# hydradarpa/kalman-hydra

Hardware: AMD Instinct MI355X
Metric: frames/sec (Brox flow + EKF update) at 1024^2 (higher is better)
Workload: dtype f32 (flow, renders) / f64 (EKF sums and state)

## Files before the change

### include/hydra_mi.h

```cpp
#ifndef HYDRA_MI_H
#define HYDRA_MI_H

#include <stdint.h>

#ifdef __cplusplus
extern "C" {
#endif

#define HM_OK 0
#define HM_ERR_ARG (-1)
#define HM_ERR_HIP (-2)
#define HM_ERR_STATE (-3)
#define HM_ERR_NUMERIC (-4)

const char *hm_last_error(void);
const char *hm_version(void);
int hm_device_count(void);

int hm_dev_alloc(int device, uint64_t bytes, void **out);
int hm_dev_free(int device, void *ptr);
int hm_dev_upload(int device, void *dst, const void *src, uint64_t bytes);
int hm_dev_download(int device, void *dst, const void *src, uint64_t bytes);
int hm_copy_stream_create(int device, void **stream_out);
int hm_copy_stream_destroy(int device, void *stream);
// ... 80 lines not shown
                  double reltol, int info[4], double *errs, double *Hzc, double *gains, double *W_out);
int hm_cov_fetch(hm_ctx_t h, double *W_out);
int hm_ms_newton(int n_vertices, int n_bars, const int32_t *bars, const double *l0, double kappa, double M,
                 double dt, int maxiter, double tol, double *X, int *newton_iterations);
int hm_ms_worker_create(void **worker);
int hm_ms_worker_destroy(void *worker);
int hm_ms_newton_start(void *worker, int n_vertices, int n_bars, const int32_t *bars, const double *l0, double kappa,
                       double M, double dt, int maxiter, double tol, const double *X);
int hm_ms_newton_finish(void *worker, double *X, int *newton_iterations);
int hm_ms_worker_attach(void *worker, hm_ctx_t ctx);
int hm_newton_dev_start(hm_ctx_t h, int N, int n_bars, const int32_t *bars, const double *l0, double kappa, double M,
                        double dt, int maxiter, double tol, const double *X);
int hm_newton_dev_finish(hm_ctx_t h, double *X, int *newton_iterations);
int hm_update_arm_newton(hm_ctx_t h, void *worker, int n_bars, const int32_t *bars, const double *l0, double kappa,
                         double M, double dt, int maxiter, double tol);
int hm_update_arm_cov(hm_ctx_t h, double eps_F);
int hm_predict_take(hm_ctx_t h, const double *X, int n_bars, const int32_t *bars, const double *l0, double kappa,
                    double a, double s, double eps_F);
int hm_cov_predict(hm_ctx_t h, const double *W_in, int n_bars, const int32_t *bars, const double *blocks,
                   double a, double s, double eps_F, double *W_out);
int hm_ms_predict(hm_ctx_t h, int n_bars, const int32_t *bars, const double *l0, double kappa, double M, double dt,
                  int maxiter, double tol, double eps_F, double *X, int *newton_iterations, int prefactor);
int hm_update_last_error(hm_ctx_t h, const double *X, double err[4]);
int hm_chain_project(hm_ctx_t h);
int hm_prepare_mask(hm_ctx_t h, const uint8_t *d_y_m);
int hm_update_arm_mask(hm_ctx_t h, const uint8_t *d_y_m);
int hm_update_tail(hm_ctx_t h, double *Hzc, double *gains);
int hm_chain_states(hm_ctx_t h, double *predicted, double *projected, int *newton_iterations, int *moved);
int hm_ctx_tune(hm_ctx_t h, const char *key, int value);
int hm_ctx_tune64(hm_ctx_t h, const char *key, int64_t value);
int hm_ctx_sync(hm_ctx_t h);
void *hm_ctx_stream(hm_ctx_t h);

typedef struct hm_smooth *hm_smooth_t;
int hm_smooth_create(hm_ctx_t ctx, int capacity, int n_bars, const int32_t *bars, const double *l0, double kappa,
                     double a, double s, double eps_F, hm_smooth_t *out);
int hm_smooth_destroy(hm_smooth_t sm);
int hm_smooth_record(hm_smooth_t sm, const double *X);
int hm_smooth_run(hm_smooth_t sm, int want_cov, double *xs, double *var);
int hm_smooth_count(hm_smooth_t sm, int *frames, int *capacity);
int hm_smooth_fetch(hm_smooth_t sm, int k, double *P_out, double *x_out, double *m_out);
int hm_smooth_prior(hm_smooth_t sm, int k, double *Pp_out);
int hm_op_smooth_gemm(int device, int which, int n, const double *A, const double *B, const double *C, double *out);

int hm_view(hm_ctx_t h, const double *X, int which, const int32_t *palette, uint8_t *bgr);
int hm_view_dev(hm_ctx_t h, const double *X, int which, const int32_t *palette, void *d_bgr, void *stream);
// ... 118 lines not shown
```

### kalman-hydra_amd/_lib.py

```python
import ctypes
import os

import numpy as np

_HERE = os.path.dirname(os.path.abspath(__file__))
SO_PATH = os.environ.get("HYDRA_MI_SO") or os.path.join(_HERE, "libhydra_mi.so")

c_f32p = ctypes.POINTER(ctypes.c_float)
c_f64p = ctypes.POINTER(ctypes.c_double)
c_u8p = ctypes.POINTER(ctypes.c_uint8)
c_i32p = ctypes.POINTER(ctypes.c_int32)
c_vp = ctypes.c_void_p

SIGNATURES = {
    "hm_last_error": (ctypes.c_char_p, []),
    "hm_version": (ctypes.c_char_p, []),
    "hm_device_count": (ctypes.c_int, []),
    "hm_dev_alloc": (ctypes.c_int, [ctypes.c_int, ctypes.c_uint64, ctypes.POINTER(c_vp)]),
    "hm_dev_free": (ctypes.c_int, [ctypes.c_int, c_vp]),
    "hm_dev_upload": (ctypes.c_int, [ctypes.c_int, c_vp, c_vp, ctypes.c_uint64]),
    "hm_dev_download": (ctypes.c_int, [ctypes.c_int, c_vp, c_vp, ctypes.c_uint64]),
    "hm_copy_stream_create": (ctypes.c_int, [ctypes.c_int, ctypes.POINTER(c_vp)]),
    "hm_copy_stream_destroy": (ctypes.c_int, [ctypes.c_int, c_vp]),
    "hm_copy_stream_sync": (ctypes.c_int, [ctypes.c_int, c_vp]),
# ... 31 lines not shown
    "hm_op_sor": (ctypes.c_int, [c_vp, c_vp, ctypes.POINTER(c_vp), ctypes.c_int, ctypes.c_int, ctypes.c_int,
                                 ctypes.c_int, ctypes.c_float]),
    "hm_ctx_create": (ctypes.c_int, [ctypes.c_int, ctypes.c_int, ctypes.c_int, ctypes.c_int, ctypes.c_int, c_vp,
                                     c_vp, ctypes.c_double, ctypes.c_double, ctypes.c_double, ctypes.POINTER(c_vp)]),
    "hm_ctx_destroy": (ctypes.c_int, [c_vp]),
    "hm_set_texture": (ctypes.c_int, [c_vp, c_vp]),
    "hm_set_observation": (ctypes.c_int, [c_vp, c_vp, c_vp, c_vp, c_vp]),
    "hm_set_observation_dev": (ctypes.c_int, [c_vp, c_vp, c_vp, c_vp, c_vp]),
    "hm_render": (ctypes.c_int, [c_vp, c_vp, c_vp, c_vp, c_vp, c_vp]),
    "hm_initjacobian": (ctypes.c_int, [c_vp, c_vp, ctypes.c_int]),
    "hm_jz": (ctypes.c_int, [c_vp, c_vp, ctypes.c_int, c_f64p, c_f64p]),
    "hm_j": (ctypes.c_int, [c_vp, c_vp, ctypes.c_double, ctypes.c_int, ctypes.c_int, c_f64p]),
    "hm_jz_multi": (ctypes.c_int, [c_vp, c_vp, ctypes.c_int, c_vp, ctypes.c_int, c_vp, c_vp]),
    "hm_j_multi": (ctypes.c_int, [c_vp, c_vp, ctypes.c_double, ctypes.c_int, c_vp, c_vp, ctypes.c_int, c_vp, c_vp, c_vp]),
    "hm_error": (ctypes.c_int, [c_vp, c_vp, ctypes.c_int, c_f64p, c_vp, c_vp]),
    "hm_measure": (ctypes.c_int, [c_vp, c_vp, ctypes.c_double, ctypes.c_int, c_vp, c_vp, c_vp]),
    "hm_update_begin": (ctypes.c_int, [c_vp, c_vp, c_vp]),
    "hm_update_step": (ctypes.c_int, [c_vp, c_vp, ctypes.c_double, ctypes.c_int, c_vp, c_vp, c_f64p]),
    "hm_update_cov": (ctypes.c_int, [c_vp, ctypes.c_int, c_vp]),
    "hm_update_prefactor": (ctypes.c_int, [c_vp]),
    "hm_update_run": (ctypes.c_int, [c_vp, c_vp, c_vp, ctypes.c_double, ctypes.c_int, ctypes.c_int, ctypes.c_double,
                                     ctypes.POINTER(ctypes.c_int), c_vp, c_vp, c_vp, c_vp]),
    "hm_update_last_error": (ctypes.c_int, [c_vp, c_vp, c_f64p]),
    "hm_cov_fetch": (ctypes.c_int, [c_vp, c_vp]),
    "hm_project_mask": (ctypes.c_int, [c_vp, c_vp, c_vp, c_vp]),
    "hm_cov_predict": (ctypes.c_int, [c_vp, c_vp, ctypes.c_int, c_vp, c_vp, ctypes.c_double, ctypes.c_double,
                                      ctypes.c_double, c_vp]),
    "hm_ms_newton": (ctypes.c_int, [ctypes.c_int, ctypes.c_int, c_vp, c_vp, ctypes.c_double, ctypes.c_double,
                                    ctypes.c_double, ctypes.c_int, ctypes.c_double, c_vp, ctypes.POINTER(ctypes.c_int)]),
    "hm_ms_worker_create": (ctypes.c_int, [ctypes.POINTER(c_vp)]),
    "hm_ms_worker_destroy": (ctypes.c_int, [c_vp]),
    "hm_ms_newton_start": (ctypes.c_int, [c_vp, ctypes.c_int, ctypes.c_int, c_vp, c_vp, ctypes.c_double, ctypes.c_double,
                                          ctypes.c_double, ctypes.c_int, ctypes.c_double, c_vp]),
    "hm_ms_newton_finish": (ctypes.c_int, [c_vp, c_vp, ctypes.POINTER(ctypes.c_int)]),
    "hm_ms_worker_attach": (ctypes.c_int, [c_vp, c_vp]),
    "hm_newton_dev_start": (ctypes.c_int, [c_vp, ctypes.c_int, ctypes.c_int, c_vp, c_vp, ctypes.c_double, ctypes.c_double,
                                           ctypes.c_double, ctypes.c_int, ctypes.c_double, c_vp]),
    "hm_newton_dev_finish": (ctypes.c_int, [c_vp, c_vp, ctypes.POINTER(ctypes.c_int)]),
    "hm_prune_mask": (ctypes.c_int, [c_vp, c_vp, c_vp]),
    "hm_chain_project": (ctypes.c_int, [c_vp]),
    "hm_prepare_mask": (ctypes.c_int, [c_vp, c_vp]),
    "hm_update_arm_mask": (ctypes.c_int, [c_vp, c_vp]),
    "hm_update_tail": (ctypes.c_int, [c_vp, c_vp, c_vp]),
    "hm_chain_states": (ctypes.c_int, [c_vp, c_vp, c_vp, ctypes.POINTER(ctypes.c_int), ctypes.POINTER(ctypes.c_int)]),
    "hm_update_arm_newton": (ctypes.c_int, [c_vp, c_vp, ctypes.c_int, c_vp, c_vp, ctypes.c_double, ctypes.c_double,
                                            ctypes.c_double, ctypes.c_int, ctypes.c_double]),
# ... 203 lines not shown
```

### kalman-hydra_amd/csrc/ctx.h

```cpp
#pragma once
#include "hm_common.h"
#include "hm_types.h"
#include <chrono>
#include <cmath>
#include <condition_variable>
#include <functional>
#include <mutex>
#include <thread>
#include <vector>

struct Helper {
    std::thread th;
    std::mutex m;
    std::condition_variable cv;
    std::function<int()> job;
    bool posted = false, busy = false, quit = false;
    int rc = HM_OK;
    char err[512] = "";
    void run()
    {
        std::unique_lock<std::mutex> lk(m);
        for (;;) {
            cv.wait(lk, [&] { return quit || posted; });
            if (quit) return;
// ... 24 lines not shown
        rc = HM_OK;
        return r;
    }
    void stop()
    {
        {
            std::unique_lock<std::mutex> lk(m);
            cv.wait(lk, [&] { return !busy; });
            quit = true;
            cv.notify_all();
        }
        if (th.joinable()) th.join();
    }
};

struct Armed {
    bool newton = false;
    void *worker = nullptr;
    bool cov = false;
    const uint8_t *mask = nullptr;
};

struct ViewState {
    Targets targets = {nullptr, nullptr, nullptr, nullptr};
    TriSetup *setup = nullptr;
    int *ids = nullptr, *lab = nullptr;
    unsigned *wire = nullptr, *mm = nullptr;
    double *X = nullptr, *force = nullptr;
    uint8_t *out = nullptr;
    hipEvent_t ev = nullptr;
    int c_layers = 0, c_L = 0;
    bool c_weighted = false;
    int *c_lab = nullptr;
    uint16_t *c_w = nullptr;
    uint8_t *c_col = nullptr;
    uint8_t *c_outline = nullptr;
    uint8_t *c_frame = nullptr;
    uint8_t *c_in = nullptr;
    uint8_t *c_slot[4] = {nullptr, nullptr, nullptr, nullptr};
    hipEvent_t c_slot_ev[4] = {nullptr, nullptr, nullptr, nullptr};
    bool c_slot_used[4] = {false, false, false, false};
    int c_next = 0;
};
#define VIEW_CELL_SLOTS 4

struct BodyState {
    bool ready = false;
// ... 92 lines not shown
    std::vector<double> resv, tailv;
    int result_delay = 0;
    bool tail_pending = false;
    bool tail_valid = false;
    long long tail_ticket = 0;
    hipStream_t tail_stream = nullptr;
    Armed armed;
    std::vector<int> sp_h_off, sp_h_bar, sp_h_other;
    std::vector<double> sp_h_blk;
    std::vector<int32_t> sp_bars_cached;
    std::vector<int> tri;
    DPool pool;
    int *d_area;
    int *d_sp_off, *d_sp_bar, *d_sp_other;
    double *d_sp_blk;
    bool upd_open;
    bool prefactored;
    std::vector<double> h_partial;
    int red_blocks = 512;
    double *d_tpart = nullptr;
    std::vector<double> h_tpart;
    int ntiles = 0;
    int render_rows = RI_H;
    bool last_err_valid = false;
    double last_err[4] = {0, 0, 0, 0};
    std::vector<double> last_err_X;
    long long run_ticket;
    int vsplit = 5, esplit;
    std::vector<int32_t> pn_bars;
    std::vector<double> pn_l0;
    double pn_par[4] = {0, 0, 0, 0};
    int pn_maxiter = 0;
    double pq_eps_F = 0.0;
    bool pq_valid = false;
    std::vector<double> pq_X, pq_l0;
    std::vector<int32_t> pq_bars;
    double pq_par[4] = {0, 0, 0, 0};
    hipStream_t stream3 = nullptr;
    int *d_n4nbr = nullptr, *d_n4nbb = nullptr, *d_n4bars = nullptr;
    double *d_n4l0 = nullptr;
    int n4deg = 0;
    std::vector<int32_t> n4_bars;
    std::vector<double> n4_l0;
    double *pin_n4 = nullptr;
    double *d_n4X = nullptr;
    std::vector<double> n4v;
// ... 30 lines not shown
    std::vector<double> h_lout;
    int2 *d_outline;
    int *d_outline_cnt;
    uint8_t *d_pm_mask;
    uint8_t *d_pm_flag = nullptr;
    uint8_t *d_pm_pruned = nullptr;
    Ccl ccl = {nullptr, nullptr, nullptr, nullptr, nullptr, 0, 0};
    double *d_pm_X = nullptr;
    double *pin_pm = nullptr;
    std::vector<double> pmv;
    int *d_pm_done = nullptr;
    long long pm_ticket = 0;
    bool pm_ready = false;
    bool outline_ready = false;
    const uint8_t *prepared_mask = nullptr;
    hipEvent_t ev_outline = nullptr;
    hipEvent_t ev_m0 = nullptr;
    ViewState view;
    BodyState body;
    StrainState strain;
    RecState rec;
};

static inline hipError_t alloc_targets(HmOwner &own, Targets &t, size_t n)
{
    hipError_t e = own.alloc(&t.acc, n * sizeof(int));
    if (e == hipSuccess) e = own.alloc(&t.fx, n * sizeof(float));
    if (e == hipSuccess) e = own.alloc(&t.fy, n * sizeof(float));
    if (e == hipSuccess) e = own.alloc(&t.cnt, n * sizeof(int));
    return e;
}

static int helper_join(hm_ctx *h)
{
    if (h->helper_used) {
        const int rc = h->helper.wait();
        if (rc != HM_OK) { hm_set_error("%s", h->helper.err); return rc; }
    }
    return HM_OK;
}
static int ctx_join(hm_ctx *h, bool lazy = false)
{
    if (!h) return HM_OK;
    if (const int rc = helper_join(h)) return rc;
    if (!lazy && h->tail_on_stream4) {
        h->tail_on_stream4 = false;
        if (hipSetDevice(h->device) != hipSuccess || hipStreamWaitEvent(h->stream, h->ev_tail, 0) != hipSuccess) {
            hm_set_error("the handle's stream cannot wait for the tail of the last update");
            return HM_ERR_HIP;
        }
    }
    if (h->worker_active) {
// ... 94 lines not shown
```

### kalman-hydra_amd/csrc/ekf.hip

```cpp
#include "ctx.h"
#include "ekf_kernels.h"
#include "dense_kernels.h"
#include "chol_flow_kernels.h"
#include "project_kernels.h"
#include "predict_kernels.h"
#include <algorithm>
#include <atomic>
#include <chrono>
#include <cmath>
#include <cstring>
#include <set>
#include <thread>
#include <utility>
#include <vector>


static int hb_wait(hipStream_t st, const double *blk, size_t first, size_t n, unsigned long long stamp, double *out, const char *who)
{
    const volatile unsigned long long *canary = (const volatile unsigned long long *)blk + 2 * (first + n - 1);
    const auto t_start = std::chrono::steady_clock::now();
    const auto t_yield = t_start + std::chrono::microseconds(700), t_give_up = t_start + std::chrono::milliseconds(20);
    bool polite = false;
    for (int spin = 0;; spin++) {
        if ((canary[0] ^ canary[1]) == stamp && hb_take(blk, first, n, stamp, out)) return HM_OK;
// ... 129 lines not shown
    hipError_t e = hipSuccess;
    auto dev = [&](auto **p, size_t bytes) { if (e == hipSuccess) e = h->own.alloc(p, bytes); };
    if (rc == HM_OK) {
        const char *pe = getenv("HYDRA_MI_EKF_PRIORITY");
        e = h->own.stream(&h->stream, !(pe && atoi(pe) == 0));
        dev(&h->d_tex, n);
        dev(&h->d_yim, n);
        dev(&h->d_ym, n);
        dev(&h->d_yfx, n * sizeof(float));
        dev(&h->d_yfy, n * sizeof(float));
        dev(&h->d_yfxm, n * sizeof(float));
        dev(&h->d_yfym, n * sizeof(float));
        dev(&h->d_setup, (size_t)T * sizeof(TriSetup));
        dev(&h->d_cfgs, (size_t)N * MEAS_NCFG * (EKF_MAX_STAR + 1) * sizeof(TriSetup));
        dev(&h->d_ubox, (size_t)N * UBOX_STRIDE * sizeof(int4));
        dev(&h->d_tmask, (size_t)N * TMASK_STRIDE * sizeof(unsigned));
        dev(&h->d_tlist, (size_t)N * TMASK_STRIDE * sizeof(int));
        dev(&h->d_tcount, (size_t)N * sizeof(int));
        dev(&h->d_X, (size_t)4 * N * sizeof(double));
        dev(&h->d_out, (size_t)h->njobs * MEAS_VSPLIT_MAX * MEAS_OUT * sizeof(double));
        dev(&h->d_partial, (size_t)h->red_blocks * 4 * sizeof(double));
        h->ntiles = hm_cdiv(W, RI_W) * hm_cdiv(H, 8);
        dev(&h->d_tpart, (size_t)h->ntiles * RI_NV * sizeof(double));
        dev(&h->d_im8, n);
        dev(&h->d_m8, n);
        const size_t n4 = (size_t)4 * N, nn = n4 * n4 * sizeof(double);
        dev(&h->d_H, nn);
        dev(&h->d_HTH, nn);
        if (e == hipSuccess) e = hipMemsetAsync(h->d_HTH, 0, nn, h->stream);
        dev(&h->d_invW0, nn);
        const size_t nn_aug = (size_t)(hm_cdiv((int)n4, DNB) * DNB + DNB) * n4 * sizeof(double);
        dev(&h->d_Af[0], nn_aug);
        dev(&h->d_Af[1], nn_aug);
        dev(&h->d_Awork, nn_aug);
        const size_t ld_bytes = (size_t)hm_cdiv((int)n4, DNB) * DNB * DNB * sizeof(double);
        dev(&h->d_T[0], nn);
        dev(&h->d_T[1], nn);
        dev(&h->d_step, n4 * sizeof(double));
        dev(&h->d_Lt[0], ld_bytes);
        dev(&h->d_Lt[1], ld_bytes);
        dev(&h->d_Wtmp, nn);
        dev(&h->d_flowP, 3 * ld_bytes);
        dev(&h->d_flowctl, 4 * sizeof(unsigned));
        if (e == hipSuccess) e = hipMemsetAsync(h->d_flowctl, 0, 4 * sizeof(unsigned), h->stream);
        dev(&h->d_Hz, n4 * sizeof(double));
        dev(&h->d_Hzc, n4 * 4 * sizeof(double));
        dev(&h->d_Wprior, nn);
        dev(&h->d_gain, n4 * 3 * sizeof(double));
        h->pin_n = 2 * (n4 + RES_HEAD + n4 * 4 + n4 * 3) + 2;
        if (e == hipSuccess) e = h->own.host_alloc(&h->pin, h->pin_n * sizeof(double), hipHostMallocCoherent);
        if (e == hipSuccess) memset(h->pin, 0, h->pin_n * sizeof(double));
        h->pin_scratch = (int *)(h->pin + h->pin_n - 2);
        h->resv.assign(n4 + RES_HEAD, 0.0);
        h->tailv.assign(n4 * 7, 0.0);
        dev(&h->d_X0, n4 * sizeof(double));
        dev(&h->pool.hdr, (size_t)4 * N * sizeof(int));
        dev(&h->pool.overflow, sizeof(int));
        dev(&h->d_area, (size_t)N * sizeof(int));
        h->pool.area = h->d_area;
        if (e == hipSuccess) e = pool_alloc(h, (long long)8 * W * H);
        dev(&h->d_Xn, n4 * sizeof(double));
        for (Targets *t : {&h->ref, &h->P, &h->Q})
            if (e == hipSuccess) e = alloc_targets(h->own, *t, n);
    }
    if (e != hipSuccess) {
        hm_set_error("hm_ctx_create: device allocation failed: %s", hipGetErrorString(e));
        step(HM_ERR_HIP);
    }
    if (rc != HM_OK) {
        ctx_free(h);
        return rc;
    }
    h->h_partial.resize((size_t)h->red_blocks * 4);
    h->h_tpart.resize((size_t)h->ntiles * RI_NV);
    *out = h;
    return HM_OK;
}

extern "C" int hm_ctx_destroy(hm_ctx_t h) { return ctx_free(h); }

void ekf_queue_setup_all(hipStream_t st, const Mesh &m, const double *d_X, TriSetup *d_setup)
{
    hipLaunchKernelGGL(k_setup_all, dim3(hm_cdiv(m.T, 64)), dim3(64), 0, st, m, d_X, d_setup);
}
void ekf_queue_render(hipStream_t st, const Mesh &m, const double *d_X, const TriSetup *d_setup, const Targets &out,
                      const int *d_labels, int *d_ids)
// ... 11 lines not shown
    return HM_OK;
}
#endif

#define TUNE_SET(field) [](hm_ctx *h, long long v) { h->field = (decltype(h->field))v; }
static const struct TuneKey {
    const char *key;
    long long lo, hi;
    int step;
    void (*set)(hm_ctx *, long long);
    const char *must;
} tune_keys[] = {
    {"measure_split", 1, MEAS_VSPLIT_MAX, 1, TUNE_SET(vsplit), nullptr},
    {"edge_split", 1, MEAS_VSPLIT_MAX, 1, TUNE_SET(esplit), nullptr},
    {"chol_flow", 0, 1, 1, TUNE_SET(chol_flow), "must be 0 (one launch per block step) or 1 (one persistent launch)"},
    {"chol_flow_wgs", 2, 2048, 1, TUNE_SET(flow_wgs), "must be in 2..2048 (the chain workgroup and at least one task workgroup)"},
    {"render_rows", 8, 16, 8, TUNE_SET(render_rows), "must be 8 or 16"},
    {"chol_flow_stall", 0, 100000, 1, TUNE_SET(flow_stall), nullptr},
    {"result_delay", 0, 5000, 1, TUNE_SET(result_delay), "must be in 0..5000 (microseconds)"},
    {"tail_async", 0, 1, 1, TUNE_SET(tail_async), "must be 0 or 1"},
    {"tail_split", 0, 1, 1, TUNE_SET(tail_split), "must be 0 or 1"},
    {"newton_fail", 0, 1, 1, TUNE_SET(newton_fail), "must be 0 or 1"},
    {"speculate", 0, 1, 1, TUNE_SET(speculate), "must be 0 or 1"},
    {"body_stats_cap", 1, BODY_STATS_CAP, 1, TUNE_SET(body.stats_cap), nullptr},
    {"body_rec_chunk", 0, INT32_MAX, 1, TUNE_SET(rec.chunk), "must be >= 0 (0: the default size)"},
    {"rec_tp_frames", 1, REC_TP_MAX, 1, TUNE_SET(rec.tp_frames), nullptr},
    {"rec_bl_frames", 1, REC_BL_MAX, 1, TUNE_SET(rec.bl_frames), nullptr},
    {"rec_res_frames", 1, REC_RES_MAX, 1, TUNE_SET(rec.res_frames), nullptr},
    {"rec_map_frames", 1, REC_MAP_MAX, 1, TUNE_SET(rec.map_frames), nullptr},
    {"rec_null_frames", 1, REC_NULL_MAX, 1, TUNE_SET(rec.null_frames), nullptr},
    {"rec_tm_frames", 1, REC_TM_MAX, 1, TUNE_SET(rec.tm_frames), nullptr},
    {"rec_gram_bytes", 64, REC_GRAM_BYTES_MAX, 64, TUNE_SET(rec.gram_bytes), "must be a multiple of 64 in 64..131008"},
    {"rec_scratch_bytes", 1, 1 << 30, 1, TUNE_SET(rec.scr_bytes), nullptr},
    {"rec_ev_bytes", 1, 1ll << 34, 1, TUNE_SET(rec.ev_bytes), nullptr},
};
#undef TUNE_SET
static const TuneKey *tune_find(const char *key)
{
    for (const TuneKey &k : tune_keys)
        if (!strcmp(key, k.key)) return &k;
    return nullptr;
}
static int tune_set(hm_ctx *h, const char *key, long long value)
{
    const TuneKey *k = tune_find(key);
    HM_ARG(k != nullptr, "hm_ctx_tune: unknown key '%s'", key);
// ... 78 lines not shown
    h->pm_ready = true;
    return HM_OK;
}
static int queue_outline(hm_ctx *h, const uint8_t *mask)
{
    HM_HIP(hipMemsetAsync(h->d_outline_cnt, 0, 4 * sizeof(int), h->stream2));
    const dim3 cg(hm_cdiv(h->W, 64), hm_cdiv(h->H, CCL_NT / 64)), cb(CCL_NT);
    hipLaunchKernelGGL(k_ccl_local, dim3(hm_cdiv(h->W, CCL_TW), hm_cdiv(h->H, CCL_TH)), cb, 0, h->stream2, mask, h->ccl);
    hipLaunchKernelGGL(k_ccl_border, cg, cb, 0, h->stream2, mask, h->ccl);
    hipLaunchKernelGGL(k_ccl_roots, cg, cb, 0, h->stream2, h->ccl);
    hipLaunchKernelGGL(k_ccl_flatten, cg, cb, 0, h->stream2, mask, h->ccl);
    hipLaunchKernelGGL(k_ccl_stats, cg, cb, 0, h->stream2, mask, h->ccl);
    hipLaunchKernelGGL(k_ccl_select, cg, cb, 0, h->stream2, mask, h->ccl);
    hipLaunchKernelGGL(k_ccl_write, cg, cb, 0, h->stream2, mask, h->ccl, h->d_pm_pruned);
    Outline o = {h->d_outline, h->d_outline_cnt, h->W * h->H, h->d_pm_flag};
    hipLaunchKernelGGL(k_outline, dim3(hm_cdiv(h->W, 64), hm_cdiv(h->H, OUTLINE_NT / 64)), dim3(OUTLINE_NT), 0, h->stream2,
                       (const uint8_t *)h->d_pm_pruned, h->W, h->H, o);
    HM_HIP(hipGetLastError());
    HM_HIP(hipEventRecord(h->ev_outline, h->stream2));
    h->prepared_mask = nullptr;
    return HM_OK;
}

static int finish_observation(hm_ctx *h)
{
    h->last_err_valid = false;
    const int n = h->W * h->H;
    hipLaunchKernelGGL(k_mask_flow, dim3(hm_cdiv(n, 256)), dim3(256), 0, h->stream, h->o_ym, h->o_yfx, h->o_yfy,
                       h->d_yfxm, h->d_yfym, n);
    HM_HIP(hipGetLastError());
    h->have_obs = true;
    return HM_OK;
}

extern "C" int hm_set_observation(hm_ctx_t h, const uint8_t *y_im, const float *y_fx, const float *y_fy,
                                  const uint8_t *y_m)
{
    HM_ARG(h && y_im && y_fx && y_fy && y_m, "hm_set_observation: NULL argument");
    HM_JOIN(h);
    HM_HIP(hipSetDevice(h->device));
    const size_t n = (size_t)h->W * h->H;
    HM_HIP(hipMemcpyAsync(h->d_yim, y_im, n, hipMemcpyHostToDevice, h->stream));
    HM_HIP(hipMemcpyAsync(h->d_ym, y_m, n, hipMemcpyHostToDevice, h->stream));
    HM_HIP(hipMemcpyAsync(h->d_yfx, y_fx, n * sizeof(float), hipMemcpyHostToDevice, h->stream));
    HM_HIP(hipMemcpyAsync(h->d_yfy, y_fy, n * sizeof(float), hipMemcpyHostToDevice, h->stream));
    h->o_yim = h->d_yim; h->o_ym = h->d_ym; h->o_yfx = h->d_yfx; h->o_yfy = h->d_yfy;
    HM_TRY(finish_observation(h));
    HM_HIP(hipStreamSynchronize(h->stream));
    h->outline_ready = false;
// ... 6 lines not shown

extern "C" int hm_set_observation_dev(hm_ctx_t h, const uint8_t *d_y_im, const float *d_y_fx, const float *d_y_fy,
                                      const uint8_t *d_y_m)
{
    HM_ARG(h && d_y_im && d_y_fx && d_y_fy && d_y_m, "hm_set_observation_dev: NULL argument");
    HM_JOIN_LAZY(h);
    HM_HIP(hipSetDevice(h->device));
    h->o_yim = d_y_im; h->o_ym = d_y_m; h->o_yfx = d_y_fx; h->o_yfy = d_y_fy;
    HM_TRY(finish_observation(h));
    h->outline_ready = false;
    if (h->d_outline && h->prepared_mask == d_y_m) {
        h->outline_ready = true;
    } else if (h->d_outline) {
        HM_TRY(queue_outline(h, h->o_ym));
        h->outline_ready = true;
    }
    h->prepared_mask = nullptr;
    return HM_OK;
}

static int render_dev(hm_ctx *h, const double *dX, Targets t)
{
    Mesh m = {h->W, h->H, h->N, h->T, h->d_tri, h->d_uv, h->d_tex};
    hipLaunchKernelGGL(k_setup_all, dim3(hm_cdiv(h->T, 64)), dim3(64), 0, h->stream, m, dX, h->d_setup);
    hipLaunchKernelGGL((k_render<0>), dim3(hm_cdiv(h->W, EKF_TILE), hm_cdiv(h->H, EKF_TILE)), dim3(EKF_TILE, EKF_TILE), 0,
                       h->stream, m, dX, h->d_setup, t, (const int *)nullptr, (int *)nullptr);
    HM_HIP(hipGetLastError());
    return HM_OK;
}

static int render_into(hm_ctx *h, const double *X, Targets t)
{
    HM_HIP(hipMemcpyAsync(h->d_X, X, (size_t)4 * h->N * sizeof(double), hipMemcpyHostToDevice, h->stream));
    return render_dev(h, h->d_X, t);
}

static void measure_args(hm_ctx *h, const double *dX, double deltaX, int masked, MeasureArgs &a);
static int render_strips(const hm_ctx *h) { return hm_cdiv(h->W, RI_W) * hm_cdiv(h->H, h->render_rows); }

static int render_iter(hm_ctx *h, const double *dX, Targets t, bool with_err, int masked, bool regions, double deltaX)
{
    IterRenderArgs r;
    r.m = Mesh{h->W, h->H, h->N, h->T, h->d_tri, h->d_uv, h->d_tex};
    r.X = dX;
    r.out = t;
    r.o = Obs{h->o_yim, masked ? h->d_yfxm : h->o_yfx, masked ? h->d_yfym : h->o_yfy, h->o_ym};
    r.raw_fx = h->o_yfx; r.raw_fy = h->o_yfy;
    r.partial = h->d_tpart;
    r.tiles_x = hm_cdiv(h->W, RI_W); r.tiles_y = hm_cdiv(h->H, h->render_rows);
    const int nstrips = r.tiles_x * r.tiles_y;
    r.with_err = with_err ? 1 : 0;
    r.n_regions = regions ? h->N : 0;
    MeasureArgs a;
    measure_args(h, dX, deltaX, masked, a);
    if (h->render_rows == 8) hipLaunchKernelGGL((k_render_iter<8>), dim3(r.n_regions + nstrips), dim3(256), 0, h->stream, r, a, h->d_area);
    else hipLaunchKernelGGL((k_render_iter<16>), dim3(r.n_regions + nstrips), dim3(256), 0, h->stream, r, a, h->d_area);
    HM_HIP(hipGetLastError());
    return HM_OK;
}

static void hm_tile_partial_sums(const double *p, int ntiles, double s[RI_NV])
{
    static thread_local double g[RI_GROUPS][RI_NV];
    for (int t = 0; t < RI_GROUPS; t++) {
        double a[RI_NV];
        for (int k = 0; k < RI_NV; k++) a[k] = 0.0;
        for (int i = t; i < ntiles; i += RI_GROUPS)
            for (int k = 0; k < RI_NV; k++) a[k] += p[RI_NV * (size_t)i + k];
        for (int k = 0; k < RI_NV; k++) g[t][k] = a[k];
    }
    for (int k = 0; k < RI_NV; k++) {
        double v = 0.0;
        for (int t = 0; t < RI_GROUPS; t++) v += g[t][k];
        s[k] = v;
    }
// ... 111 lines not shown
                const int v = h->tri[3 * t + k];
                const double x = states[sidx][2 * v], y = states[sidx][2 * v + 1];
                x0 = std::min(x0, x); x1 = std::max(x1, x); y0 = std::min(y0, y); y1 = std::max(y1, y);
            }
        if (!(x0 <= x1 && y0 <= y1)) continue;
        const int c0 = (int)std::max(0.0, std::floor(std::min(x0, (double)h->W)) - 1.0);
        const int c1 = (int)std::min((double)h->W - 1.0, std::ceil(std::max(x1, -1.0)) + 1.0);
        const int r0 = (int)std::max(0.0, std::floor(std::min(y0, (double)h->H)) - 1.0);
        const int r1 = (int)std::min((double)h->H - 1.0, std::ceil(std::max(y1, -1.0)) + 1.0);
        int4 &b = box[lab];
        if (b.x > b.y) b = make_int4(c0, c1, r0, r1);
        else b = make_int4(std::min(b.x, c0), std::max(b.y, c1), std::min(b.z, r0), std::max(b.w, r1));
    }
    HM_HIP(hipMemcpyAsync(h->d_labels, labels, (size_t)h->T * sizeof(int), hipMemcpyHostToDevice, h->stream));
    HM_HIP(hipMemcpyAsync(h->d_lbox, box.data(), (size_t)n_labels * sizeof(int4), hipMemcpyHostToDevice, h->stream));
    HM_HIP(hipStreamSynchronize(h->stream));
    return HM_OK;
}

static int render_ids(hm_ctx *h, const double *X, Targets t, int *ids, bool ids_only)
{
    HM_HIP(hipMemcpyAsync(h->d_X, X, (size_t)4 * h->N * sizeof(double), hipMemcpyHostToDevice, h->stream));
    Mesh m = {h->W, h->H, h->N, h->T, h->d_tri, h->d_uv, h->d_tex};
    hipLaunchKernelGGL(k_setup_all, dim3(hm_cdiv(h->T, 64)), dim3(64), 0, h->stream, m, h->d_X, h->d_setup);
    const dim3 grid(hm_cdiv(h->W, EKF_TILE), hm_cdiv(h->H, EKF_TILE)), block(EKF_TILE, EKF_TILE);
    if (ids_only) hipLaunchKernelGGL((k_render<2>), grid, block, 0, h->stream, m, h->d_X, h->d_setup, t, (const int *)h->d_labels, ids);
    else hipLaunchKernelGGL((k_render<1>), grid, block, 0, h->stream, m, h->d_X, h->d_setup, t, (const int *)h->d_labels, ids);
    HM_HIP(hipGetLastError());
    HM_HIP(hipStreamSynchronize(h->stream));
    return HM_OK;
}

extern "C" int hm_jz_multi(hm_ctx_t h, const double *Xp, int masked, const int32_t *labels, int n_labels, double *hz,
                           double *hzc)
{
    HM_ARG(h && Xp && labels && hz && n_labels >= 1, "hm_jz_multi: bad argument");
    HM_JOIN(h);
    NEED_REF(h, "hm_jz_multi");
    HM_HIP(hipSetDevice(h->device));
    const double *states[2] = {h->X0.data(), Xp};
    HM_TRY(multi_setup(h, labels, n_labels, states, 2));
    int rc = render_ids(h, h->X0.data(), h->ref, h->d_ids[0], true);
    if (rc == HM_OK) rc = render_ids(h, Xp, h->P, h->d_ids[1], false);
    if (rc) return rc;
    MultiArgs a = {h->ref, h->P, h->P, h->d_ids[0], h->d_ids[1], h->d_ids[1], obs_of(h, masked), h->W, h->d_lbox, h->d_lout};
    hipLaunchKernelGGL(k_jz_multi, dim3(n_labels), dim3(RED_NT), 0, h->stream, a);
// ... 837 lines not shown
        HM_TRY(update_queue_iteration(u, it, swap));
        HM_TRY(update_meanwhile(u, it));
        Taken taken = Taken::go_on;
        HM_TRY(update_take_result(u, it, swap, &taken));
        if (taken == Taken::retry) continue;
        Verdict verdict = Verdict::go_on;
        HM_TRY(update_judge(u, it, &verdict));
        if (verdict != Verdict::go_on) break;
        swap.keep();
        it++;
    }
    HM_TRY(update_state_final(u));
    HM_TRY(update_tail(u));
    update_finish(u, info);
    return HM_OK;
}

extern "C" int hm_update_last_error(hm_ctx_t h, const double *X, double err[4])
{
    HM_ARG(h && X && err, "hm_update_last_error: NULL argument");
    if (!h->last_err_valid || h->last_err_X.size() != (size_t)4 * h->N) return 1;
    if (memcmp(X, h->last_err_X.data(), (size_t)4 * h->N * sizeof(double)) != 0) return 1;
    for (int k = 0; k < 4; k++) err[k] = h->last_err[k];
    return HM_OK;
}

void ekf_queue_fpft(hipStream_t st, const double *src, double *FP, double *dst, int N, const SpringTopo &tp, double a, double s,
                    double eps_F)
{
    const dim3 grid(hm_cdiv(4 * N, 256), N);
    hipLaunchKernelGGL(k_fw_rows, grid, dim3(256), 0, st, src, FP, N, tp, a, s);
    hipLaunchKernelGGL(k_pft_cols, grid, dim3(256), 0, st, (const double *)FP, dst, N, tp, a, s, eps_F);
}
void ekf_queue_chol_flow(hipStream_t st, const FlowArgs &a, int wgs, bool fill)
{
    if (fill) hipLaunchKernelGGL(k_flow_fill, dim3(a.nrows + FLOW_FILL_WGS), dim3(256), 0, st, a);
    hipLaunchKernelGGL(k_chol_flow, dim3(wgs), dim3(FLOW_NT), 0, st, a);
}

static int cov_predict_core(hm_ctx *h, const double *W_in, int n_bars, const int32_t *bars, const double *blocks,
                            double a, double s, double eps_F, double *W_out, bool ahead, hipStream_t st = nullptr)
{
    if (!st) st = h->stream;
    const int N = h->N, n4 = 4 * N;
    const size_t nn = (size_t)n4 * n4 * sizeof(double);
    std::vector<int> &off = h->sp_h_off, &bar = h->sp_h_bar, &other = h->sp_h_other;
// ... 320 lines not shown
```

### kalman-hydra_amd/csrc/ekf_kernels.h

```cpp
#pragma once
#include <hip/hip_runtime.h>
#include <stdint.h>
#include "hm_types.h"

__global__ void k_setup_all(Mesh m, const double *__restrict__ X, TriSetup *__restrict__ out)
{
    int t = blockIdx.x * blockDim.x + threadIdx.x;
    if (t >= m.T) return;
    int v0 = m.tri[3 * t], v1 = m.tri[3 * t + 1], v2 = m.tri[3 * t + 2];
    TriSetup s;
    d_tri_setup(s, v0, v1, v2, d_snap(X[2 * v0]), d_snap(X[2 * v0 + 1]), d_snap(X[2 * v1]), d_snap(X[2 * v1 + 1]),
                d_snap(X[2 * v2]), d_snap(X[2 * v2 + 1]), m.W, m.H);
    d_tri_attr(s, m.uv, X, m.N);
    out[t] = s;
}

template <int MODE>
__global__ __launch_bounds__(EKF_TILE *EKF_TILE) void k_render(Mesh m, const double *__restrict__ X,
                                                                const TriSetup *__restrict__ setup, Targets out,
                                                                const int *__restrict__ labels, int *__restrict__ ids)
{
    __shared__ unsigned s_mask[EKF_MAX_TRI / 32];
    const int tid = threadIdx.y * EKF_TILE + threadIdx.x;
    const int words = (m.T + 31) / 32;
// ... 702 lines not shown
                acc[B_VXX] = fma(avx, bxfx, acc[B_VXX]); acc[B_VXY] = fma(avx, byfx, acc[B_VXY]);
                acc[B_VXVX] = fma(avx, bvx, acc[B_VXVX]);
                acc[B_XVY] = fma(axfy, bvy, acc[B_XVY]); acc[B_YVY] = fma(ayfy, bvy, acc[B_YVY]);
                acc[B_VYX] = fma(avy, bxfy, acc[B_VYX]); acc[B_VYY] = fma(avy, byfy, acc[B_VYY]);
                acc[B_VYVY] = fma(avy, bvy, acc[B_VYVY]);
            }
            if (!more) break;
        }
    }
    d_block_reduce<B_NV, MEAS_NT>(acc, s_red, a.out + ((size_t)(N + e) * MEAS_VSPLIT_MAX + blockIdx.y) * MEAS_OUT);
}

#define RI_CHUNK 32
#define RI_GROUPS 256
#define RI_W 64
struct IterRenderArgs {
    Mesh m;
    const double *X;
    Targets out;
    Obs o;
    const float *raw_fx, *raw_fy;
    double *partial;
    int tiles_x, tiles_y, with_err, n_regions;
};
#define RI_NV 6
struct RenderShared {
    unsigned mask[EKF_MAX_TRI / 32];
    TriSetup cand[RI_CHUNK];
    double red[(256 / 64) * RI_NV];
    unsigned band[RI_W / 8];
};

#ifdef HM_STAMP
__device__ long long *g_stamp;
#define HM_STAMP_AT(k) do { if (g_stamp && threadIdx.x == 0) g_stamp[(size_t)blockIdx.x * 8 + (k)] = wall_clock64(); } while (0)
#else
#define HM_STAMP_AT(k) do { } while (0)
#endif
template <int RIH>
__global__ __launch_bounds__(256, 4) void k_render_iter(IterRenderArgs r, MeasureArgs a, int *__restrict__ area)
{
    HM_STAMP_AT(0);
    constexpr int RI_PX = RI_W * RIH / 256;
    __shared__ union {
        RegionShared reg;
        RenderShared t;
// ... 16 lines not shown
        const bool has2 = tc < m.T;
        const int a0 = m.tri[3 * ta], a1 = m.tri[3 * ta + 1], a2 = m.tri[3 * ta + 2];
        const int b0 = has2 ? m.tri[3 * tc] : a0, b1 = has2 ? m.tri[3 * tc + 1] : a1, b2 = has2 ? m.tri[3 * tc + 2] : a2;
        const double ax0 = X[2 * a0], ay0 = X[2 * a0 + 1], ax1 = X[2 * a1], ay1 = X[2 * a1 + 1], ax2 = X[2 * a2], ay2 = X[2 * a2 + 1];
        const double bx0 = X[2 * b0], by0 = X[2 * b0 + 1], bx1 = X[2 * b1], by1 = X[2 * b1 + 1], bx2 = X[2 * b2], by2 = X[2 * b2 + 1];
#pragma unroll
        for (int k = 0; k < 2; k++) {
            if (k == 1 && !has2) break;
            const int t = k ? tc : ta;
            const double x0 = k ? bx0 : ax0, y0 = k ? by0 : ay0, x1 = k ? bx1 : ax1, y1 = k ? by1 : ay1, x2 = k ? bx2 : ax2, y2 = k ? by2 : ay2;
            const double lo_x = fmin(x0, fmin(x1, x2)) - 2.0, hi_x = fmax(x0, fmax(x1, x2)) + 2.0;
            const double lo_y = fmin(y0, fmin(y1, y2)) - 2.0, hi_y = fmax(y0, fmax(y1, y2)) + 2.0;
            if (hi_x < (double)c0 || lo_x > (double)(c0 + RI_W) || hi_y < (double)r0 || lo_y > (double)(r0 + RIH)) continue;
            int cmin, cmax, rmin, rmax;
            d_tri_bbox(d_snap(x0), d_snap(y0), d_snap(x1), d_snap(y1), d_snap(x2), d_snap(y2), m.W, m.H, cmin, cmax, rmin, rmax);
            if (cmin <= cmax && cmax >= c0 && cmin < c0 + RI_W && rmax >= r0 && rmin < r0 + RIH)
                atomicOr(&sh.t.mask[t >> 5], 1u << (t & 31));
        }
    }
    __syncthreads();
    HM_STAMP_AT(1);
    int total = 0;
    for (int w = 0; w < words; w++) total += __popc(sh.t.mask[w]);
    const int c = c0 + (tid & 63), rb = r0 + (tid >> 6);
    int acc[RI_PX], cnt[RI_PX], tadr[RI_PX];
    float fx[RI_PX], fy[RI_PX];
#pragma unroll
    for (int q = 0; q < RI_PX; q++) { acc[q] = 0; cnt[q] = 0; fx[q] = 0.0f; fy[q] = 0.0f; tadr[q] = -1; }
    for (int base = 0; base < total; base += RI_CHUNK) {
        const int nch = min(RI_CHUNK, total - base);
        for (int tb = tid; tb < m.T; tb += 256) {
            const unsigned word = sh.t.mask[tb >> 5], bit = 1u << (tb & 31);
            if (!(word & bit)) continue;
            int rank = __popc(word & (bit - 1u));
            for (int w = 0; w < (tb >> 5); w++) rank += __popc(sh.t.mask[w]);
            if (rank < base || rank >= base + nch) continue;
            const int v0 = m.tri[3 * tb], v1 = m.tri[3 * tb + 1], v2 = m.tri[3 * tb + 2];
            TriSetup su;
            d_tri_setup(su, v0, v1, v2, d_snap(X[2 * v0]), d_snap(X[2 * v0 + 1]), d_snap(X[2 * v1]), d_snap(X[2 * v1 + 1]),
                        d_snap(X[2 * v2]), d_snap(X[2 * v2 + 1]), m.W, m.H);
            d_tri_attr(su, m.uv, X, m.N);
            {
                const double xa = (double)c0, xb = (double)min(c0 + RI_W - 1, m.W - 1);
                const double ya = (double)r0, yb = (double)min(r0 + RIH - 1, m.H - 1);
                bool out = false;
#pragma unroll
// ... 39 lines not shown
                    if (tadr[j] < 0) tadr[j] = at;
                    else acc[j] += m.tex[at];
                    fx[j] = fx[j] + d_lerp(su.ax[0], su.ax[1], su.ax[2], l1, l2);
                    fy[j] = fy[j] + d_lerp(su.ay[0], su.ay[1], su.ay[2], l1, l2);
                    cnt[j]++;
                }
            }
        __syncthreads();
    }
    HM_STAMP_AT(2);
    {
        int tx[RI_PX];
#pragma unroll
        for (int j = 0; j < RI_PX; j++) tx[j] = m.tex[tadr[j] < 0 ? 0 : tadr[j]];
#pragma unroll
        for (int j = 0; j < RI_PX; j++) acc[j] += tadr[j] < 0 ? 0 : tx[j];
    }
    double e[RI_NV] = {0.0, 0.0, 0.0, 0.0, 0.0, 0.0};
#pragma unroll
    for (int j = 0; j < RI_PX; j++) {
        const int rr = rb + 4 * j;
        if (c >= m.W || rr >= m.H) continue;
        const int p = rr * m.W + c;
        r.out.acc[p] = acc[j]; r.out.fx[p] = fx[j]; r.out.fy[p] = fy[j]; r.out.cnt[p] = cnt[j];
        if (r.with_err) {
            const unsigned rim = acc[j] > 255 ? 255 : acc[j];
            const unsigned rm = cnt[j] > 0 ? 255 : 0;
            const unsigned d = ((unsigned)r.o.yim[p] - rim) & 255u;
            const unsigned dm = ((255u * (unsigned)r.o.ym[p]) - rm) & 255u;
            const float dfx = r.o.yfx[p] - fx[j];
            const float dfy = r.o.yfy[p] + fy[j];
            e[0] += (double)((d * d) & 255u);
            e[1] += (double)dfx * (double)dfx;
            e[2] += (double)dfy * (double)dfy;
            e[3] += (double)((dm * dm) & 255u);
            const float gfx = r.raw_fx[p] - fx[j];
            const float gfy = r.raw_fy[p] + fy[j];
            e[4] += (double)gfx * (double)gfx;
            e[5] += (double)gfy * (double)gfy;
        }
    }
    HM_STAMP_AT(3);
    if (!r.with_err) return;
    d_block_reduce<RI_NV, 256>(e, sh.t.red, r.partial + RI_NV * (size_t)tile);
    HM_STAMP_AT(4);
}

__device__ __forceinline__ void d_tile_partial_sums(const double *__restrict__ partial, int ntiles, double *sp, double *out)
{
    const int t = threadIdx.x;
    if (t < RI_GROUPS) {
        double s[RI_NV];
#pragma unroll
        for (int k = 0; k < RI_NV; k++) s[k] = 0.0;
#pragma unroll 4
        for (int i = t; i < ntiles; i += RI_GROUPS) {
            const double2 *q = (const double2 *)(partial + RI_NV * (size_t)i);
#pragma unroll
            for (int k = 0; k < RI_NV / 2; k++) { const double2 v = q[k]; s[2 * k] += v.x; s[2 * k + 1] += v.y; }
        }
#pragma unroll
        for (int k = 0; k < RI_NV; k++) sp[RI_NV * t + k] = s[k];
    }
    __syncthreads();
    if (t < RI_NV) {
        double s = 0.0;
// ... 92 lines not shown
```

### kalman-hydra_amd/csrc/hm_types.h

```cpp
#pragma once
#include <hip/hip_runtime.h>
#include <stdint.h>
#include <stddef.h>


#define EKF_SUB 256
#define EKF_MAX_STAR 24
#define EKF_TILE 16
#define EKF_MAX_TRI 4096

struct TriSetup {
    double ea[3], eb[3], ec[3];
    double ecb[3];
    int cmin, cmax, rmin, rmax;
    int tl[3];
    float inv;
    int i0, i1, i2;
    float ux[3], uy[3], ax[3], ay[3];
};

__device__ __forceinline__ void d_tri_attr(TriSetup &s, const float *__restrict__ uv, const double *__restrict__ X, int N)
{
    const int id[3] = {s.i0, s.i1, s.i2};
    for (int k = 0; k < 3; k++) {
// ... 114 lines not shown
    float ty = d_lerp(s.uy[0], s.uy[1], s.uy[2], l1, l2);
    int cx = (int)floorf(tx), cy = (int)floorf(ty);
    cx = cx < 0 ? 0 : (cx > W - 1 ? W - 1 : cx);
    cy = cy < 0 ? 0 : (cy > H - 1 ? H - 1 : cy);
    return cy * W + cx;
}
__device__ __forceinline__ int d_texel(const uint8_t *__restrict__ tex, const TriSetup &s, float l1, float l2, int W,
                                       int H)
{
    return tex[d_texel_at(s, l1, l2, W, H)];
}

struct Mesh {
    int W, H, N, T;
    const int *tri;
    const float *uv;
    const uint8_t *tex;
};

struct Targets {
    int *acc;
    float *fx, *fy;
    int *cnt;
};

struct DPool {
    int *hdr;
    int *live;
    const int *area;
    short2 *xi, *yi;
    float *xfx, *xfy, *yfx, *yfy, *vxfx, *vyfy;
    long long cap;
    int *overflow;
};

#define RI_H 16

#define DNB 32

typedef double d4_t __attribute__((ext_vector_type(4)));

__device__ __forceinline__ d4_t d_mfma_nn(double (*X)[DNB + 1], double (*Y)[DNB + 1], int wv, int lane, d4_t c)
{
    const int i = 16 * (wv >> 1) + (lane & 15), j = 16 * (wv & 1) + (lane & 15), kq = lane >> 4;
#pragma unroll
    for (int kk = 0; kk < DNB / 4; kk++)
// ... 83 lines not shown
```

### kalman-hydra_amd/renderer.py

```python
import ctypes
import os

import numpy as np

from . import _lib
from . import matio


class ChainedPredictionFailed(RuntimeError):
    """hm_update_run, chained to a state prediction on the device (hm_chain_project), found that the prediction's inner
    solve had given up: nothing was updated; predict on the host and update again."""


class Renderer:
    def __init__(self, distmesh, vel, flow, nx, im1, cuda, eps_Z, eps_J, eps_M, labels=None, labels_hess=None,
                 Q=None, showtracking=False, force=None, multi=True, device=0):
        if not cuda:
            raise NotImplementedError(
                "cuda=False: this build has no CPU measurement path (the reference's NumPy twin, "
                "cuda.py:929-1010, is restated under oracle/ as test infrastructure only)")
        self._h = None
        self.Q = Q
        self.cuda = cuda
        self.force = force
# ... 50 lines not shown
        self.velocities = np.asarray(velocities, np.float64).reshape(-1, 2)
        table = self.labels_hess if hess else self.labels
        if multi_idx is None or multi_idx < 0 or table is None:
            self._palette = None
        else:
            self._palette = np.ascontiguousarray(np.asarray(table)[:, multi_idx], np.int32)

    def _X(self, state=None):
        if state is not None:
            return np.ascontiguousarray(np.asarray(state.X, np.float64).reshape(-1))
        return np.ascontiguousarray(np.concatenate((self.vertices.reshape(-1), self.velocities.reshape(-1))))

    def render(self):
        n = self.nx * self.ny
        im = np.empty((self.ny, self.nx), np.uint8)
        m = np.empty_like(im)
        fx = np.empty((self.ny, self.nx), np.float32)
        fy = np.empty_like(fx)
        _lib.check(_lib.lib().hm_render(self._h, _lib.ptr(self._X()), _lib.ptr(im), _lib.ptr(fx), _lib.ptr(fy),
                                        _lib.ptr(m)), "hm_render")
        self.last_render = (im, fx, fy, m)
        return self.last_render

    def get_flow(self):
        _, fx, fy, _ = self.render()
        return fx, fy

    def _view_palette(self):
        lh = self.labels_hess
        if lh is None or np.ndim(lh) != 2 or np.shape(lh)[1] < 2:
            return None
        return np.ascontiguousarray(np.asarray(lh)[:, 1], np.int32)

    def view(self, X=None, which="overlay"):
        from .videoio import VIEWS
        x = self._X() if X is None else np.ascontiguousarray(np.asarray(X, np.float64).reshape(-1))
        if x.shape[0] != 4 * self.n:
            raise ValueError("state of %d entries for a mesh of %d vertices" % (x.shape[0], self.n))
        out = np.empty((self.ny, self.nx, 3), np.uint8)
        pal = self._view_palette() if which == "mask" else None
        _lib.check(_lib.lib().hm_view(self._h, _lib.ptr(x), VIEWS[which], _lib.ptr(pal), _lib.ptr(out)), "hm_view")
        return out

    def view_dev(self, X, which, d_out, stream=None):
        from .videoio import VIEWS
        x = np.ascontiguousarray(np.asarray(X, np.float64).reshape(-1))
# ... 863 lines not shown
```

Before: 335.8.

## Skip rewriting empty render tiles and reuse per-tile error partials across iterations

```diff
diff --git a/include/hydra_mi.h b/include/hydra_mi.h
--- a/include/hydra_mi.h
+++ b/include/hydra_mi.h
@@ -126,6 +126,7 @@
 int hm_ms_predict(hm_ctx_t h, int n_bars, const int32_t *bars, const double *l0, double kappa, double M, double dt,
                   int maxiter, double tol, double eps_F, double *X, int *newton_iterations, int prefactor);
 int hm_update_last_error(hm_ctx_t h, const double *X, double err[4]);
+int hm_targets_fetch(hm_ctx_t h, int which, int32_t *acc, float *fx, float *fy, int32_t *cnt);
 int hm_chain_project(hm_ctx_t h);
 int hm_prepare_mask(hm_ctx_t h, const uint8_t *d_y_m);
 int hm_update_arm_mask(hm_ctx_t h, const uint8_t *d_y_m);
diff --git a/kalman-hydra_amd/_lib.py b/kalman-hydra_amd/_lib.py
--- a/kalman-hydra_amd/_lib.py
+++ b/kalman-hydra_amd/_lib.py
@@ -77,6 +77,7 @@
     "hm_update_run": (ctypes.c_int, [c_vp, c_vp, c_vp, ctypes.c_double, ctypes.c_int, ctypes.c_int, ctypes.c_double,
                                      ctypes.POINTER(ctypes.c_int), c_vp, c_vp, c_vp, c_vp]),
     "hm_update_last_error": (ctypes.c_int, [c_vp, c_vp, c_f64p]),
+    "hm_targets_fetch": (ctypes.c_int, [c_vp, ctypes.c_int, c_vp, c_vp, c_vp, c_vp]),
     "hm_cov_fetch": (ctypes.c_int, [c_vp, c_vp]),
     "hm_project_mask": (ctypes.c_int, [c_vp, c_vp, c_vp, c_vp]),
     "hm_cov_predict": (ctypes.c_int, [c_vp, c_vp, ctypes.c_int, c_vp, c_vp, ctypes.c_double, ctypes.c_double,
diff --git a/kalman-hydra_amd/csrc/ctx.h b/kalman-hydra_amd/csrc/ctx.h
--- a/kalman-hydra_amd/csrc/ctx.h
+++ b/kalman-hydra_amd/csrc/ctx.h
@@ -70,7 +70,7 @@
 };
 
 struct ViewState {
-    Targets targets = {nullptr, nullptr, nullptr, nullptr};
+    Targets targets = {nullptr, nullptr, nullptr, nullptr, nullptr};
     TriSetup *setup = nullptr;
     int *ids = nullptr, *lab = nullptr;
     unsigned *wire = nullptr, *mm = nullptr;
@@ -209,6 +209,11 @@
     std::vector<double> h_tpart;
     int ntiles = 0;
     int render_rows = RI_H;
+    int render_skip = 1;
+    int *d_tstamp = nullptr;
+    int obs_epoch = 1;
+    bool skip_live = false;
+    int skip_rows = 0, skip_masked = -1;
     bool last_err_valid = false;
     double last_err[4] = {0, 0, 0, 0};
     std::vector<double> last_err_X;
@@ -285,12 +290,13 @@
     RecState rec;
 };
 
-static inline hipError_t alloc_targets(HmOwner &own, Targets &t, size_t n)
+static inline hipError_t alloc_targets(HmOwner &own, Targets &t, size_t n, size_t strips = 0)
 {
     hipError_t e = own.alloc(&t.acc, n * sizeof(int));
     if (e == hipSuccess) e = own.alloc(&t.fx, n * sizeof(float));
     if (e == hipSuccess) e = own.alloc(&t.fy, n * sizeof(float));
     if (e == hipSuccess) e = own.alloc(&t.cnt, n * sizeof(int));
+    if (e == hipSuccess && strips) e = own.alloc(&t.dirty, strips);
     return e;
 }
 
diff --git a/kalman-hydra_amd/csrc/ekf.hip b/kalman-hydra_amd/csrc/ekf.hip
--- a/kalman-hydra_amd/csrc/ekf.hip
+++ b/kalman-hydra_amd/csrc/ekf.hip
@@ -175,6 +175,7 @@
         dev(&h->d_partial, (size_t)h->red_blocks * 4 * sizeof(double));
         h->ntiles = hm_cdiv(W, RI_W) * hm_cdiv(H, 8);
         dev(&h->d_tpart, (size_t)h->ntiles * RI_NV * sizeof(double));
+        dev(&h->d_tstamp, (size_t)h->ntiles * sizeof(int));
         dev(&h->d_im8, n);
         dev(&h->d_m8, n);
         const size_t n4 = (size_t)4 * N, nn = n4 * n4 * sizeof(double);
@@ -214,7 +215,7 @@
         if (e == hipSuccess) e = pool_alloc(h, (long long)8 * W * H);
         dev(&h->d_Xn, n4 * sizeof(double));
         for (Targets *t : {&h->ref, &h->P, &h->Q})
-            if (e == hipSuccess) e = alloc_targets(h->own, *t, n);
+            if (e == hipSuccess) e = alloc_targets(h->own, *t, n, (size_t)h->ntiles);
     }
     if (e != hipSuccess) {
         hm_set_error("hm_ctx_create: device allocation failed: %s", hipGetErrorString(e));
@@ -272,6 +273,7 @@
     {"tail_split", 0, 1, 1, TUNE_SET(tail_split), "must be 0 or 1"},
     {"newton_fail", 0, 1, 1, TUNE_SET(newton_fail), "must be 0 or 1"},
     {"speculate", 0, 1, 1, TUNE_SET(speculate), "must be 0 or 1"},
+    {"render_skip", 0, 1, 1, TUNE_SET(render_skip), "must be 0 or 1"},
     {"body_stats_cap", 1, BODY_STATS_CAP, 1, TUNE_SET(body.stats_cap), nullptr},
     {"body_rec_chunk", 0, INT32_MAX, 1, TUNE_SET(rec.chunk), "must be >= 0 (0: the default size)"},
     {"rec_tp_frames", 1, REC_TP_MAX, 1, TUNE_SET(rec.tp_frames), nullptr},
@@ -396,9 +398,20 @@
     return HM_OK;
 }
 
+static void obs_epoch_bump(hm_ctx *h)
+{
+    if (h->obs_epoch == INT32_MAX) h->skip_live = false;
+    else h->obs_epoch++;
+}
+static hipError_t targets_all_dirty(hm_ctx *h, const Targets &t)
+{
+    return t.dirty ? hipMemsetAsync(t.dirty, 1, (size_t)h->ntiles, h->stream) : hipSuccess;
+}
+
 static int finish_observation(hm_ctx *h)
 {
     h->last_err_valid = false;
+    obs_epoch_bump(h);
     const int n = h->W * h->H;
     hipLaunchKernelGGL(k_mask_flow, dim3(hm_cdiv(n, 256)), dim3(256), 0, h->stream, h->o_ym, h->o_yfx, h->o_yfy,
                        h->d_yfxm, h->d_yfym, n);
@@ -451,6 +464,7 @@
 static int render_dev(hm_ctx *h, const double *dX, Targets t)
 {
     Mesh m = {h->W, h->H, h->N, h->T, h->d_tri, h->d_uv, h->d_tex};
+    HM_HIP(targets_all_dirty(h, t));
     hipLaunchKernelGGL(k_setup_all, dim3(hm_cdiv(h->T, 64)), dim3(64), 0, h->stream, m, dX, h->d_setup);
     hipLaunchKernelGGL((k_render<0>), dim3(hm_cdiv(h->W, EKF_TILE), hm_cdiv(h->H, EKF_TILE)), dim3(EKF_TILE, EKF_TILE), 0,
                        h->stream, m, dX, h->d_setup, t, (const int *)nullptr, (int *)nullptr);
@@ -480,6 +494,18 @@
     const int nstrips = r.tiles_x * r.tiles_y;
     r.with_err = with_err ? 1 : 0;
     r.n_regions = regions ? h->N : 0;
+    if (h->render_skip && with_err && masked != h->skip_masked) { obs_epoch_bump(h); h->skip_masked = masked; }
+    if (h->render_skip && (!h->skip_live || h->skip_rows != h->render_rows)) {
+        for (const Targets *q : {&h->ref, &h->P, &h->Q}) HM_HIP(targets_all_dirty(h, *q));
+        HM_HIP(hipMemsetAsync(h->d_tstamp, 0, (size_t)h->ntiles * sizeof(int), h->stream));
+        h->obs_epoch = 1;
+        h->skip_rows = h->render_rows;
+        h->skip_live = true;
+    }
+    if (!h->render_skip) h->skip_live = false;
+    r.skip = h->render_skip;
+    r.stamp = h->d_tstamp;
+    r.epoch = h->obs_epoch;
     MeasureArgs a;
     measure_args(h, dX, deltaX, masked, a);
     if (h->render_rows == 8) hipLaunchKernelGGL((k_render_iter<8>), dim3(r.n_regions + nstrips), dim3(256), 0, h->stream, r, a, h->d_area);
@@ -637,6 +663,7 @@
 {
     HM_HIP(hipMemcpyAsync(h->d_X, X, (size_t)4 * h->N * sizeof(double), hipMemcpyHostToDevice, h->stream));
     Mesh m = {h->W, h->H, h->N, h->T, h->d_tri, h->d_uv, h->d_tex};
+    if (!ids_only) HM_HIP(targets_all_dirty(h, t));
     hipLaunchKernelGGL(k_setup_all, dim3(hm_cdiv(h->T, 64)), dim3(64), 0, h->stream, m, h->d_X, h->d_setup);
     const dim3 grid(hm_cdiv(h->W, EKF_TILE), hm_cdiv(h->H, EKF_TILE)), block(EKF_TILE, EKF_TILE);
     if (ids_only) hipLaunchKernelGGL((k_render<2>), grid, block, 0, h->stream, m, h->d_X, h->d_setup, t, (const int *)h->d_labels, ids);
@@ -1520,6 +1547,21 @@
     if (!h->last_err_valid || h->last_err_X.size() != (size_t)4 * h->N) return 1;
     if (memcmp(X, h->last_err_X.data(), (size_t)4 * h->N * sizeof(double)) != 0) return 1;
     for (int k = 0; k < 4; k++) err[k] = h->last_err[k];
+    return HM_OK;
+}
+
+extern "C" int hm_targets_fetch(hm_ctx_t h, int which, int32_t *acc, float *fx, float *fy, int32_t *cnt)
+{
+    HM_ARG(h != nullptr && (which == 0 || which == 1), "hm_targets_fetch: NULL handle or which not 0 / 1");
+    HM_JOIN(h);
+    HM_HIP(hipSetDevice(h->device));
+    const Targets &t = which ? h->P : h->ref;
+    const size_t n = (size_t)h->W * h->H;
+    if (acc) HM_HIP(hipMemcpyAsync(acc, t.acc, n * sizeof(int), hipMemcpyDeviceToHost, h->stream));
+    if (fx) HM_HIP(hipMemcpyAsync(fx, t.fx, n * sizeof(float), hipMemcpyDeviceToHost, h->stream));
+    if (fy) HM_HIP(hipMemcpyAsync(fy, t.fy, n * sizeof(float), hipMemcpyDeviceToHost, h->stream));
+    if (cnt) HM_HIP(hipMemcpyAsync(cnt, t.cnt, n * sizeof(int), hipMemcpyDeviceToHost, h->stream));
+    HM_HIP(hipStreamSynchronize(h->stream));
     return HM_OK;
 }
 
diff --git a/kalman-hydra_amd/csrc/ekf_kernels.h b/kalman-hydra_amd/csrc/ekf_kernels.h
--- a/kalman-hydra_amd/csrc/ekf_kernels.h
+++ b/kalman-hydra_amd/csrc/ekf_kernels.h
@@ -748,6 +748,8 @@
     const float *raw_fx, *raw_fy;
     double *partial;
     int tiles_x, tiles_y, with_err, n_regions;
+    int *stamp;
+    int skip, epoch;
 };
 #define RI_NV 6
 struct RenderShared {
@@ -810,6 +812,22 @@
     HM_STAMP_AT(1);
     int total = 0;
     for (int w = 0; w < words; w++) total += __popc(sh.t.mask[w]);
+    bool put = true, err = r.with_err != 0;
+    if (r.skip) {
+        if (__builtin_amdgcn_readfirstlane(total) == 0) {
+            put = __builtin_amdgcn_readfirstlane((int)r.out.dirty[tile]) != 0;
+            if (err) err = __builtin_amdgcn_readfirstlane(r.stamp[tile]) != r.epoch;
+            if (!put && !err) { HM_STAMP_AT(4); return; }
+            __syncthreads();
+            if (tid == 0) {
+                r.out.dirty[tile] = 0;
+                if (err) r.stamp[tile] = r.epoch;
+            }
+        } else if (tid == 0) {
+            r.out.dirty[tile] = 1;
+            if (err) r.stamp[tile] = 0;
+        }
+    }
     const int c = c0 + (tid & 63), rb = r0 + (tid >> 6);
     int acc[RI_PX], cnt[RI_PX], tadr[RI_PX];
     float fx[RI_PX], fy[RI_PX];
@@ -895,8 +913,8 @@
         const int rr = rb + 4 * j;
         if (c >= m.W || rr >= m.H) continue;
         const int p = rr * m.W + c;
-        r.out.acc[p] = acc[j]; r.out.fx[p] = fx[j]; r.out.fy[p] = fy[j]; r.out.cnt[p] = cnt[j];
-        if (r.with_err) {
+        if (put) { r.out.acc[p] = acc[j]; r.out.fx[p] = fx[j]; r.out.fy[p] = fy[j]; r.out.cnt[p] = cnt[j]; }
+        if (err) {
             const unsigned rim = acc[j] > 255 ? 255 : acc[j];
             const unsigned rm = cnt[j] > 0 ? 255 : 0;
             const unsigned d = ((unsigned)r.o.yim[p] - rim) & 255u;
@@ -914,7 +932,7 @@
         }
     }
     HM_STAMP_AT(3);
-    if (!r.with_err) return;
+    if (!err) return;
     d_block_reduce<RI_NV, 256>(e, sh.t.red, r.partial + RI_NV * (size_t)tile);
     HM_STAMP_AT(4);
 }
diff --git a/kalman-hydra_amd/csrc/hm_types.h b/kalman-hydra_amd/csrc/hm_types.h
--- a/kalman-hydra_amd/csrc/hm_types.h
+++ b/kalman-hydra_amd/csrc/hm_types.h
@@ -160,6 +160,7 @@
     int *acc;
     float *fx, *fy;
     int *cnt;
+    uint8_t *dirty;
 };
 
 struct DPool {
diff --git a/kalman-hydra_amd/renderer.py b/kalman-hydra_amd/renderer.py
--- a/kalman-hydra_amd/renderer.py
+++ b/kalman-hydra_amd/renderer.py
@@ -96,6 +96,15 @@
         self.last_render = (im, fx, fy, m)
         return self.last_render
 
+    def targets(self, which):
+        acc = np.empty((self.ny, self.nx), np.int32)
+        cnt = np.empty_like(acc)
+        fx = np.empty((self.ny, self.nx), np.float32)
+        fy = np.empty_like(fx)
+        _lib.check(_lib.lib().hm_targets_fetch(self._h, int(which), _lib.ptr(acc), _lib.ptr(fx), _lib.ptr(fy),
+                                               _lib.ptr(cnt)), "hm_targets_fetch")
+        return acc, fx, fy, cnt
+
     def get_flow(self):
         _, fx, fy, _ = self.render()
         return fx, fy
```

After: 338.5 (median of 6 runs). About the same (+0.8%).
